# Inception3D/Motion324

Measured on AMD Instinct MI355X. Metric: frames/sec (32-frame clip, 2048 pts, 512x512), higher is better.
Workload: dtype bf16; 1 GPU; Motion_Latent_Model.forward inference, B=1 x 32 frames x 2048 points x 512x512 video, 4096 surface samples, training.frames=32, random-init weights (one clip per GPU; BASELINE configs[1]); the clip sits in the replayed graph's input buffers in HBM; bf16 speed mode with the decoder's residual stream in bf16 and the head fused (no [rows, C] intermediate) (secondary.headline_without_precision_shortcu; parallelism=clip-parallel x1

## Files before the change

### include/m324.h

```cpp
#ifndef M324_H
#define M324_H

#ifdef __cplusplus
extern "C" {
#endif

typedef enum { M324_OK = 0, M324_ERR_INVALID = -1, M324_ERR_HIP = -2, M324_ERR_UNSUPPORTED = -3 } m324_status;
typedef enum { M324_F32 = 0, M324_BF16 = 1, M324_MXFP8 = 2 } m324_dtype;
typedef enum { M324_ACT_NONE = 0, M324_ACT_GELU = 1 } m324_act;
typedef enum { M324_AUX_NONE = 0, M324_AUX_STORE_PREACT = 1, M324_AUX_MUL_GELU_GRAD = 2, M324_AUX_QKV_HEADS = 3,
               M324_AUX_QKV_HEADS_VT = 4, M324_AUX_N3 = 5, M324_AUX_STORE_GELU_GRAD = 6, M324_AUX_MUL = 7 } m324_aux_mode;

int m324_abi_version(void);
int m324_last_error(char* buf, int n);
int m324_device_info(char* name, int n);
int m324_set_tunable(const char* name, int value);

typedef struct {
    const void* A;  long lda;
    const void* W;  long ldw;
    void* C;        long ldc;
    int M, N, K;
    int in_dtype, out_dtype;
    const float* bias;
// ... 5 lines not shown
    long strideA, strideW, strideC;
    void* aux; long ldaux; int aux_mode;
    void* qkv_q; void* qkv_k; void* qkv_v;
    const float* qkv_qw; const float* qkv_kw;
    float qkv_eps, qkv_qscale;
    int qkv_L, qkv_H;
    const float* ln_rowstat; const float* ln_colsum;
    float* ln_stats_out;
    void* ln_copy_out; long ln_ldcopy;
    int ln_ncb; float ln_eps;
} m324_gemm_args;
int m324_gemm(const m324_gemm_args* a, void* stream);
int m324_gemm_pair(const m324_gemm_args* a, const m324_gemm_args* b, void* stream);
int m324_gemm_plan(const m324_gemm_args* a, char* buf, int n);

int m324_mx_quant(const void* x, int x_dtype, long ldx, int rows, int K, void* q, long ldq, void* s, long lds, void* stream);
int m324_layernorm_mx(const float* x, long ldx, const float* w, const float* b, float eps, int rows, int C, void* q, long ldq,
                      void* s, long lds, void* stream);
int m324_gemm_mx(const m324_gemm_args* a, const void* A_scale, long lds_a, const void* W_scale, long lds_w, void* C_scale,
                 long lds_c, void* stream);

int m324_rowstats_finish(const float* part, int ncb, int M, float eps, float* rowstat, void* stream);
int m324_rowstats(const float* x, long ldx, int rows, int C, float eps, float* rowstat, void* copy, long ldcopy, void* stream);

int m324_n3_finish(const float* part, int ncb, int M, const float* bias3, float* out, void* stream);

int m324_gemm_tn(const void* X, long ldx, const void* Y, long ldy, float* C, long ldc, int M, int N, int Kc,
                 int slices, long strideC, void* stream);

int m324_layernorm(const float* x, long ldx, const float* w, const float* b, float eps,
                   void* y, long ldy, int out_dtype, int rows, int C,
                   int gin, int gout, int off, void* stream);
int m324_layernorm_pair(const float* x0, long ldx0, const float* w0, const float* b0, float eps0, void* y0, long ldy0, int rows0,
                        int gin0, int gout0, int off0, const float* x1, long ldx1, const float* w1, const float* b1, float eps1,
                        void* y1, long ldy1, int rows1, int gin1, int gout1, int off1, int C, int out_dtype, void* stream);
int m324_layernorm_in(const void* x, int x_dtype, long ldx, const float* w, const float* b, float eps,
                      void* y, long ldy, int out_dtype, int rows, int C,
                      int gin, int gout, int off, void* stream);

int m324_qkv_split(const void* q_src, long ldq, const void* k_src, long ldk, const void* v_src, long ldv,
                   const float* q_w, const float* k_w, float eps, float q_scale,
                   void* Q, void* K, void* V, void* Qt, void* Kt, void* Vt,
                   int B, int L, int H, int dtype, void* stream);

enum { M324_ATTN_Q_PRESCALED = 1, M324_ATTN_V_ROWMAJOR = 2, M324_ATTN_SCORES_BOUNDED = 4 };
int m324_attention(const void* Q, long q_bstride, const void* K, const void* Vt, void* O, long ldo,
// ... 100 lines not shown
```

### motion324_amd/Pcd_motion.py

```python
from __future__ import annotations

import contextlib
import os

from typing import Dict, Optional

import torch
import torch.nn as nn
import torch.nn.functional as F

from . import ops, parallel, switches
from .easydict import EasyDict as edict
from .image_encoder import DINO_EPS, DinoEncoder
from .lib import ACT_GELU, M324Error
from .loss import MSELossComputer
from .prepared import Prepared, bump_generation, compute_dtype, pad_k
from .timing import span
from . import transformer as _transformer
from .transformer import (LN_EPS, LNFold, QK_Norm_CrossAttentionBlock, QK_Norm_TransformerBlock, fusion_off, init_weights,
                          mx_scope)

AUTO_GRAPH = switches.flag("M324_AUTO_GRAPH")
FUSE_HEAD_N3 = switches.flag("M324_FUSE_HEAD")
KV_REHEARSE = int(switches.get("M324_KV_REHEARSE") or 0)
KV_OVERLAP = switches.flag("M324_KV_OVERLAP")
BF16_DECODER_STREAM = switches.flag("M324_BF16_DECODER")
HOIST_DECODER_Q = switches.flag("M324_HOIST_Q")
DECODE_ROWS = int(switches.get("M324_DECODE_ROWS"))
MXFP8_DEFAULT = switches.flag("M324_MXFP8")


def _get(cfg, key, default=None):
    if isinstance(cfg, dict):
        return cfg.get(key, default)
    return getattr(cfg, key, default)


class PointEmbed(nn.Module):

    def __init__(self, hidden_dim=48, dim=768):
        super().__init__()
        if hidden_dim != 48:
            raise NotImplementedError("m324_point_encode implements the reference's 48 Fourier features")
        self.embedding_dim = hidden_dim
        e = torch.pow(2, torch.arange(hidden_dim // 6)).float() * torch.pi
        z = torch.zeros(hidden_dim // 6)
        self.register_buffer("basis", torch.stack([torch.cat([e, z, z]), torch.cat([z, e, z]), torch.cat([z, z, e])]))
        self.mlp = nn.Linear(hidden_dim + 3, dim)


def generate_pos_embed(T: int, H: int, W: int, embed_dim: int) -> torch.Tensor:
    def axis(n):
# ... 463 lines not shown
        drop_seed = int(torch.randint(0, 2 ** 62, (1,)).item()) if drop_p > 0.0 else 0
        pos = self._video_pos(P, T_full)[t0 * Pn:(t0 + T) * Pn]
        sp_rest = P.f32(self.special_token_rest).reshape(4, C)
        sp_first = P.f32(self.special_token_0).reshape(4, C) if t0 == 0 else sp_rest
        tok = ops.assemble_tokens(dino_x, P.vec(enc.norm.weight), P.vec(enc.norm.bias), DINO_EPS, pos, sp_first, sp_rest,
                                  mesh, P.vec(self.transformer_input_layernorm.weight),
                                  self.transformer_input_layernorm.eps, B, T, K, Pn, drop_p, drop_seed)
        Lt = 4 + K + Pn
        if cap is not None:
            dn = torch.empty((B * T * Pn, C), dtype=torch.float32, device=dev)
            ops.layernorm(dino_x, P.vec(enc.norm.weight), P.vec(enc.norm.bias), DINO_EPS, dn, row_map=(Pn, Pn + 1, 1))
            cap["dino_tokens"], cap["trunk_in"] = dn, tok.clone()

        if shard is not None and parallel.collectives_on(shard[1]):
            rank, world, group = shard[:3]
            kv_gather = _KVGather(B, T, Lt, parallel.counts(T_full, world), group, dev, rank=rank)

        fold = None
        if LNFold.usable(P, tok.shape[0], C) and "trunk.mlp" not in mx.roles:
            fold = LNFold(tok)
            if "trunk.qkv" not in mx.roles:
                fold.from_stream(tok, self.global_transformer_blocks[0].norm1.eps)
        n_pairs = len(self.global_transformer_blocks)
        for i, (gblk, lblk) in enumerate(zip(self.global_transformer_blocks, self.local_transformer_blocks)):
            with mx:
                gblk.run(P, tok, B, T * Lt, kv_gather=kv_gather, fold=fold)
                lblk.run(P, tok, B * T, Lt, fold=fold, feed_next=i + 1 < n_pairs)
            if cap is not None and "trunk_block0" not in cap:
                cap["trunk_block0"] = tok.clone()
        if cap is not None:
            cap["trunk_out"] = tok.clone()

        dec = self.decoder_cross_attn
        out = torch.empty((B, T, N, 3), dtype=torch.float32, device=dev)
        head_ln, head_fc1, head_fc2 = self.shared_mlp_output[0], self.shared_mlp_output[1], self.shared_mlp_output[3]
        w3, b3 = P.f32(head_fc2.weight), P.vec(head_fc2.bias)
        nchunk = max(1, min(N, DECODE_ROWS // T))
        pcd, nrm, rgb = (self._f32c(sample[k]) for k in ("ref_pcd", "ref_normal", "ref_rgb"))
        paired = None
        if hoisted is None and B == 1 and nchunk == N:
            pf0 = self._point_features(P, pcd[0], nrm[0].contiguous(), rgb[0].contiguous())
            with span("stage:decoder_cross_attn_block", self.decoder_block_flops(B, T, N)):
                Q0, Kd, Vd = dec.project_q_kv(P, pf0, N, tok, B * T, K, row_map=(K, Lt, 4))
            paired = (pf0, Q0)
        else:
            with span("stage:decoder_cross_attn_block", self.decoder_block_flops(B, T, N)):
                Kd, Vd = dec.project_kv(P, tok, B * T, K, row_map=(K, Lt, 4))
        for b in range(B):
            for n0 in range(0, N, nchunk):
                n1 = min(N, n0 + nchunk)
                if hoisted is not None:
                    pf, Q = hoisted[b]
                elif paired is not None:
                    pf, Q = paired
                else:
                    pf = self._point_features(P, pcd[b, n0:n1], nrm[b, n0:n1].contiguous(), rgb[b, n0:n1].contiguous())
                with span("stage:decoder_cross_attn_block", 0.0):
                    x, fold_d = self.decoder_block(P, Kd[b * T:(b + 1) * T], Vd[b * T:(b + 1) * T], pf,
                                                   None if (hoisted is None and paired is None) else Q)
                if cap is not None and n0 == 0 and n1 == N:
                    cap.setdefault("decoder_out_t0", []).append(x[:N].clone())
                if fold_d is not None:
                    hw, hcs, hb = P.folded(head_ln.weight, head_ln.bias, head_fc1.weight, head_fc1.bias)
                    h, lnk = fold_d.xb, dict(ln=fold_d.ln(head_ln.eps, hcs))
                else:
                    h = torch.empty(x.shape, dtype=P.dtype, device=dev)
                    ops.layernorm(x, P.vec(head_ln.weight), P.vec(head_ln.bias), head_ln.eps, h)
                    hw, hb, lnk = P.mat(head_fc1.weight), P.vec(head_fc1.bias), {}
                whole = n0 == 0 and n1 == N
                o = out[b] if whole else torch.empty((T, n1 - n0, 3), dtype=torch.float32, device=dev)
# ... 42 lines not shown
```

### motion324_amd/csrc/elementwise.hip

```cpp
#include "common.h"

namespace {

constexpr int LN_MAXV = 4;

__device__ __forceinline__ long remap_row(long r, int gin, int gout, int off) {
    return gin > 0 ? (r / gin) * gout + (r % gin) + off : r;
}

#define LN_FOR(i, c) _Pragma("unroll") for (int i = 0, c = lane * 4; i < LN_MAXV; ++i, c += 256) if (c < C)

__device__ __forceinline__ void row_load(float4 (&v)[LN_MAXV], const float* src, int lane, int C) {
    LN_FOR(i, c) v[i] = *reinterpret_cast<const float4*>(src + c);
}
__device__ __forceinline__ void row_stats(const float4 (&v)[LN_MAXV], int lane, int C, float eps, float& mean, float& rstd) {
    float s = 0.f;
    LN_FOR(i, c) s += v[i].x + v[i].y + v[i].z + v[i].w;
    mean = wave_sum(s) / (float)C;
    float q = 0.f;
    LN_FOR(i, c) {
        float a = v[i].x - mean, b = v[i].y - mean, cc = v[i].z - mean, d = v[i].w - mean;
        q += a * a + b * b + cc * cc + d * d;
    }
    rstd = rsqrtf(wave_sum(q) / (float)C + eps);
// ... 128 lines not shown
    const float n = 64.0f * (float)ncb, mean = s / n;
    float m2 = 0.f;
    for (int b = 0; b < ncb; ++b) {
        const float2 pb = part[(long)b * M + m];
        const float d = pb.x * (1.0f / 64.0f) - mean;
        m2 += fmaf(64.0f * d, d, pb.y);
    }
    const float rstd = rsqrtf(m2 / n + eps);
    rowstat[m] = make_float2(rstd, -rstd * mean);
}

__global__ __launch_bounds__(256) void rowstats_kernel(const float* __restrict__ x, long ldx, int rows, int C, float eps,
                                                       float2* __restrict__ rowstat, bf16_t* __restrict__ copy, long ldcopy) {
    const int lane = threadIdx.x & 63;
    const long row = (long)blockIdx.x * 4 + (threadIdx.x >> 6);
    if (row >= rows) return;
    float4 v[LN_MAXV];
    row_load(v, x + row * ldx, lane, C);
    float mean, rstd;
    row_stats(v, lane, C, eps, mean, rstd);
    if (lane == 0) rowstat[row] = make_float2(rstd, -rstd * mean);
    if (copy) {
        LN_FOR(i, c) store4<bf16_t>(copy + row * ldcopy + c, v[i].x, v[i].y, v[i].z, v[i].w);
    }
}

template <typename T>
__global__ __launch_bounds__(256) void qkv_split_kernel(const T* __restrict__ qs, long ldq, const T* __restrict__ ks, long ldk,
                                                        const T* __restrict__ vs, long ldv, const float* __restrict__ qw,
                                                        const float* __restrict__ kw, float eps, float q_scale,
                                                        T* __restrict__ Q, T* __restrict__ K, T* __restrict__ V,
                                                        T* __restrict__ Qt, T* __restrict__ Kt, T* __restrict__ Vt, int L, int H,
                                                        int Lp) {
    __shared__ float tile[64][65];
    const int t = threadIdx.x, tok = t >> 2, part = t & 3;
    const int b = blockIdx.z, h = blockIdx.y, l0 = blockIdx.x * 64;
    const int l = l0 + tok;
    const bool ok = l < L;
    const long srow = (long)b * L + l;
    const long hbase = ((long)b * H + h);

    auto one = [&](const T* src, long ld, const float* w, float post, T* dst, T* dstT) {
        float v[16];
        if (ok) {
            const T* p = src + srow * ld + h * 64 + part * 16;
            float lo[8], hi8[8];
// ... 698 lines not shown
    else M324_FAIL(M324_ERR_UNSUPPORTED, name ": dtype %d", (int)(dtype))

extern "C" int m324_rowstats_finish(const float* part, int ncb, int M, float eps, float* rowstat, void* stream) {
    M324_REQUIRE(part && rowstat && ncb > 0 && M > 0, "m324_rowstats_finish: bad arguments (ncb=%d M=%d)", ncb, M);
    M324_REQUIRE(((uintptr_t)part % 8) == 0 && ((uintptr_t)rowstat % 8) == 0, "m324_rowstats_finish: tables must be 8-byte aligned");
    hipLaunchKernelGGL(rowstats_finish_kernel, dim3(ceil_div(M, 256)), dim3(256), 0, (hipStream_t)stream,
                       reinterpret_cast<const float2*>(part), ncb, M, eps, reinterpret_cast<float2*>(rowstat));
    M324_CHECK_LAUNCH("m324_rowstats_finish");
    return M324_OK;
}

extern "C" int m324_rowstats(const float* x, long ldx, int rows, int C, float eps, float* rowstat, void* copy, long ldcopy,
                             void* stream) {
    M324_REQUIRE(x && rowstat && rows > 0, "m324_rowstats: bad arguments");
    M324_REQUIRE(C % 4 == 0 && C > 0 && C <= 256 * LN_MAXV && ldx % 4 == 0 && ldx >= C, "m324_rowstats: C=%d ldx=%ld unsupported", C, ldx);
    M324_REQUIRE(((uintptr_t)rowstat % 8) == 0 && (!copy || (ldcopy % 4 == 0 && ldcopy >= C && ((uintptr_t)copy % 8) == 0)),
                 "m324_rowstats: misaligned outputs");
    hipLaunchKernelGGL(rowstats_kernel, dim3(ceil_div(rows, 4)), dim3(256), 0, (hipStream_t)stream, x, ldx, rows, C, eps,
                       reinterpret_cast<float2*>(rowstat), static_cast<bf16_t*>(copy), ldcopy);
    M324_CHECK_LAUNCH("m324_rowstats");
    return M324_OK;
}

extern "C" int m324_layernorm_in(const void* x, int x_dtype, long ldx, const float* w, const float* b, float eps, void* y, long ldy,
                                 int out_dtype, int rows, int C, int gin, int gout, int off, void* stream) {
    if (x_dtype == M324_F32) return m324_layernorm((const float*)x, ldx, w, b, eps, y, ldy, out_dtype, rows, C, gin, gout, off, stream);
    M324_REQUIRE(x && w && y, "m324_layernorm_in: null pointer");
    M324_REQUIRE(x_dtype == M324_BF16 && out_dtype == M324_BF16, "m324_layernorm_in: a bf16 input needs a bf16 output");
    M324_REQUIRE(rows > 0 && C % 4 == 0 && C > 0 && C <= 256 * LN_MAXV && ldx % 4 == 0 && ldy % 4 == 0,
                 "m324_layernorm_in: rows=%d C=%d ldx=%ld ldy=%ld unsupported", rows, C, ldx, ldy);
    if (m324::tunable(m324::TUN_LN_ROWS) == 1)
        hipLaunchKernelGGL((layernorm1_kernel<bf16_t, bf16_t>), dim3(ceil_div(rows, 4)), dim3(256), 0, (hipStream_t)stream,
                           (const bf16_t*)x, ldx, w, b, eps, (bf16_t*)y, ldy, rows, C, gin, gout, off);
    else
    hipLaunchKernelGGL((layernorm_kernel<bf16_t, bf16_t>), dim3(ceil_div(rows, 8)), dim3(256), 0, (hipStream_t)stream,
                       (const bf16_t*)x, ldx, w, b, eps, (bf16_t*)y, ldy, rows, C, gin, gout, off);
    M324_CHECK_LAUNCH("m324_layernorm_in");
    return M324_OK;
}

extern "C" int m324_layernorm(const float* x, long ldx, const float* w, const float* b, float eps, void* y, long ldy,
                              int out_dtype, int rows, int C, int gin, int gout, int off, void* stream) {
    M324_REQUIRE(x && w && y, "m324_layernorm: null pointer");
    M324_REQUIRE(rows > 0, "m324_layernorm: rows=%d", rows);
    M324_REQUIRE(C % 4 == 0 && C > 0 && C <= 256 * LN_MAXV, "m324_layernorm: C=%d unsupported", C);
    M324_REQUIRE(ldx % 4 == 0 && ldy % 4 == 0, "m324_layernorm: leading dims must be multiples of 4");
// ... 384 lines not shown
```

### motion324_amd/lib.py

```python
from __future__ import annotations

import ctypes as C
import os
import threading

HERE = os.path.dirname(os.path.abspath(__file__))
LIB_PATH = os.environ.get("M324_LIB") or os.path.join(HERE, "libm324.so")

F32, BF16, MXFP8 = 0, 1, 2
ACT_NONE, ACT_GELU = 0, 1
ABI_VERSION = 23
ERR_UNSUPPORTED = -3


class M324Error(RuntimeError):
    pass


class GemmArgs(C.Structure):
    _fields_ = [
        ("A", C.c_void_p), ("lda", C.c_long),
        ("W", C.c_void_p), ("ldw", C.c_long),
        ("C", C.c_void_p), ("ldc", C.c_long),
        ("M", C.c_int), ("N", C.c_int), ("K", C.c_int),
# ... 23 lines not shown
class MirrorItem(C.Structure):
    _fields_ = [("src_off", C.c_long), ("dst_off", C.c_long), ("dstT_off", C.c_long), ("first_tile", C.c_long), ("rows", C.c_int),
                ("cols", C.c_int), ("ldT", C.c_int), ("pad_", C.c_int)]


_P, _L, _I, _F = C.c_void_p, C.c_long, C.c_int, C.c_float

SIGNATURES = {
    "m324_abi_version": [],
    "m324_last_error": [C.c_char_p, _I],
    "m324_device_info": [C.c_char_p, _I],
    "m324_set_tunable": [C.c_char_p, _I],
    "m324_gemm": [C.POINTER(GemmArgs), _P],
    "m324_gemm_plan": [C.POINTER(GemmArgs), C.c_char_p, _I],
    "m324_gemm_pair": [C.POINTER(GemmArgs), C.POINTER(GemmArgs), _P],
    "m324_mx_quant": [_P, _I, _L, _I, _I, _P, _L, _P, _L, _P],
    "m324_layernorm_mx": [_P, _L, _P, _P, _F, _I, _I, _P, _L, _P, _L, _P],
    "m324_gemm_mx": [C.POINTER(GemmArgs), _P, _L, _P, _L, _P, _L, _P],
    "m324_attention_plan": [_I, _I, _I, _I, _I, _I, C.c_char_p, _I],
    "m324_gemm_tn": [_P, _L, _P, _L, _P, _L, _I, _I, _I, _I, _L, _P],
    "m324_n3_finish": [_P, _I, _I, _P, _P, _P],
    "m324_rowstats_finish": [_P, _I, _I, _F, _P, _P],
    "m324_rowstats": [_P, _L, _I, _I, _F, _P, _P, _L, _P],
    "m324_layernorm": [_P, _L, _P, _P, _F, _P, _L, _I, _I, _I, _I, _I, _I, _P],
    "m324_layernorm_in": [_P, _I, _L, _P, _P, _F, _P, _L, _I, _I, _I, _I, _I, _I, _P],
    "m324_layernorm_pair": [_P, _L, _P, _P, _F, _P, _L, _I, _I, _I, _I, _P, _L, _P, _P, _F, _P, _L, _I, _I, _I, _I, _I, _I, _P],
    "m324_qkv_split": [_P, _L, _P, _L, _P, _L, _P, _P, _F, _F, _P, _P, _P, _P, _P, _P, _I, _I, _I, _I, _P],
    "m324_attention": [_P, _L, _P, _P, _P, _L, _I, _I, _I, _I, _F, _I, _P, _I, _P],
    "m324_attention_merge": [_P, _P, _P, _P, _P, _P, _L, _P, _L, _I, _I, _I, _I, _P],
    "m324_patchify": [_P, _I, _I, _I, _I, _I, _P, _I, _I, _P],
    "m324_patchify_u8": [_P, _I, _I, _I, _I, _I, _P, _I, _I, _P],
    "m324_point_encode": [_P, _I, _P, _L, _I, _P],
    "m324_point_concat": [_P, _P, _I, _P, _I, _I, _I, _P],
    "m324_dino_cls_rows": [_P, _P, _P, _I, _I, _I, _P],
    "m324_assemble_tokens": [_P, _P, _P, _F, _P, _P, _P, _P, _P, _F, _P, _I, _I, _I, _I, _I, _F, C.c_ulonglong, _P],
    "m324_linear_n3": [_P, _L, _P, _P, _P, _I, _I, _I, _P],
    "m324_mse": [_P, _P, _L, _F, _P, _P, _P],
    "m324_smooth_trajectories": [_P, _P, _P, _I, _I, _I, _F, _F, _P],
    "m324_smooth_savgol": [_P, _P, _I, _I, _I, _P, _I, _P],
    "m324_smooth_oneeuro": [_P, _P, _I, _I, _I, _F, _F, _F, _P],
    "m324_nearest_point": [_P, _I, _P, _I, _P, _P],
    "m324_transpose": [_P, _L, _P, _L, _I, _I, _I, _I, _P],
    "m324_colsum": [_P, _L, _P, _I, _I, _I, _I, _P, _I, _P],
    "m324_colsum_multi": [C.POINTER(ColsumItem), _I, _P],
    "m324_gelu": [_P, _P, _L, _I, _P],
    "m324_gelu_bwd": [_P, _P, _P, _L, _I, _P],
# ... 84 lines not shown
```

### motion324_amd/ops.py

```python
from __future__ import annotations

import ctypes as C
from typing import NamedTuple, Optional

import torch

from . import lib as L
from . import switches
from .timing import active as _timing, span

F32, BF16, MXFP8 = L.F32, L.BF16, L.MXFP8
_TORCH_DT = {F32: torch.float32, BF16: torch.bfloat16}


def code_of(dtype: torch.dtype) -> int:
    if dtype == torch.float32:
        return F32
    if dtype == torch.bfloat16:
        return BF16
    raise L.M324Error(f"unsupported dtype {dtype}")


def torch_dtype(code: int) -> torch.dtype:
    return _TORCH_DT[code]
# ... 376 lines not shown
    if (two != 2 or part.dtype != torch.float32 or not part.is_contiguous() or rowstat.dtype != torch.float32
            or not rowstat.is_contiguous() or rowstat.numel() != 2 * M):
        raise L.M324Error("rowstats_finish: part [ncb, M, 2] and rowstat [M, 2] must be contiguous fp32")
    with span("hbm_pass", 0.0, 8.0 * (ncb + 1) * M, f"rowstats_finish_kernel | rows={M} blocks={ncb}" if _timing() else ""):
        L.check(L.load().m324_rowstats_finish(_p(part), ncb, M, eps, _p(rowstat), _stream()), "m324_rowstats_finish")
    return rowstat


def rowstats(x: torch.Tensor, eps: float, rowstat: torch.Tensor, copy: Optional[torch.Tensor] = None) -> torch.Tensor:
    px, ldx = _rows(x, "x")
    rows, Cdim = x.shape
    if x.dtype != torch.float32 or rowstat.dtype != torch.float32 or not rowstat.is_contiguous() or rowstat.numel() != 2 * rows:
        raise L.M324Error("rowstats: x fp32 [rows, C], rowstat contiguous fp32 [rows, 2]")
    pc, ldc = (None, 0)
    if copy is not None:
        if copy.dtype != torch.bfloat16 or copy.shape[0] < rows or copy.shape[1] != Cdim:
            raise L.M324Error("rowstats: copy must be bf16 [rows, C]")
        pc, ldc = _rows(copy, "copy")
    with span("hbm_pass", 0.0, rows * Cdim * (4.0 + (2.0 if copy is not None else 0.0)), f"rowstats_kernel | rows={rows} C={Cdim}" if _timing() else ""):
        L.check(L.load().m324_rowstats(px, ldx, rows, Cdim, eps, _p(rowstat), pc, ldc, _stream()), "m324_rowstats")
    return rowstat


def layernorm(x: torch.Tensor, w: torch.Tensor, b: Optional[torch.Tensor], eps: float, out: torch.Tensor,
              rows: Optional[int] = None, row_map=(0, 0, 0)) -> torch.Tensor:
    if x.dtype != torch.float32 and not (x.dtype == torch.bfloat16 and out.dtype == torch.bfloat16):
        raise L.M324Error("layernorm: x must be fp32 (or bf16 with a bf16 output)")
    px, ldx = _rows(x, "x")
    py, ldy = _rows(out, "out")
    Cdim = x.shape[1]
    rows = out.shape[0] if rows is None else rows
    gin, gout, off = row_map
    need = ((rows - 1) // gin * gout + (rows - 1) % gin + off + 1) if gin > 0 else rows
    if x.shape[0] < need or out.shape[0] < rows or out.shape[1] != Cdim:
        raise L.M324Error("layernorm: shape mismatch")
    tag = (f"layernorm_kernel<{'unsigned short' if out.element_size() == 2 else 'float'}, {'unsigned short' if x.element_size() == 2 else 'float'}>"
           f" | rows={rows} C={Cdim}") if _timing() else ""
    with span("hbm_pass", 0.0, float(rows) * Cdim * (x.element_size() + out.element_size()), tag):
        if x.dtype == torch.bfloat16:
            L.check(L.load().m324_layernorm_in(px, BF16, ldx, _vec(w, Cdim, "w"), _vec(b, Cdim, "b"), eps, py, ldy, code_of(out.dtype),
                                               rows, Cdim, gin, gout, off, _stream()), "m324_layernorm_in")
        else:
            L.check(L.load().m324_layernorm(px, ldx, _vec(w, Cdim, "w"), _vec(b, Cdim, "b"), eps, py, ldy, code_of(out.dtype),
                                            rows, Cdim, gin, gout, off, _stream()), "m324_layernorm")
    return out

# ... 481 lines not shown
```

### motion324_amd/switches.py

```python
from __future__ import annotations

import os
from typing import Dict, Tuple

HOST: Dict[str, Tuple[str, str, str]] = {
    "M324_AUTO_GRAPH": ("1", "Pcd_motion.AUTO_GRAPH", "inference forward(): hipGraph replay from the third call with the same shapes on"),
    "M324_FUSE_HEAD": ("1", "Pcd_motion.FUSE_HEAD_N3", "bf16 inference: head Linear + GELU + Linear(C -> 3) in one GEMM epilogue (M324_AUX_N3)"),
    "M324_BF16_DECODER": ("1", "Pcd_motion.BF16_DECODER_STREAM", "bf16 inference: the decoder's two-addition residual stream in bf16 (0: fp32 like the trunk)"),
    "M324_HOIST_Q": ("1", "Pcd_motion.HOIST_DECODER_Q", "graph capture: decoder point features + q projection on the shape-encoder branch"),
    "M324_DECODE_ROWS": (str(1 << 17), "Pcd_motion.DECODE_ROWS", "max (frames x points) rows per decoder pass"),
    "M324_OVERLAP": ("1", "Pcd_motion.OVERLAP_SHAPE_ENCODER", "inference: shape encoder on a second HIP stream under the image encoder"),
    "M324_KV_OVERLAP": ("0", "Pcd_motion.KV_OVERLAP", "frame-parallel (one sample), opt-in until it has run on a multi-GPU RCCL node: 1 = every global block attends to the rank's own keys while the k|v all-gather is in flight, then to the gathered remote keys, and merges the partial softmaxes by their log-sum-exps (0: one attention after the gather)"),
    "M324_KV_REHEARSE": ("0", "Pcd_motion.KV_REHEARSE", "one rank with forced collectives (bench.py M324_BENCH_COLLECT=1): W > 1 runs every global block's overlapped form as rank 0 of W would (own keys = the first 1 / W of the frames), to price the split attention + merge on one GPU"),
    "M324_FOLD_LN": ("2", "transformer.FOLD_LN", "LayerNorm fold: 0 off, 1 bf16 streams only (the decoder), 2 every stream (trunk, DINO too)"),
    "M324_FOLD_MERGE": ("1", "transformer.FOLD_MERGE", "LayerNorm fold: the consumer GEMM merges the producer's per-block row statistics itself (0: m324_rowstats_finish launch between them)"),
    "M324_PAIR_PROJ": ("1", "transformer.PAIR_PROJ", "bf16 inference, decoder: norm_q + norm_kv in one launch and the q + k|v projections in one launch when the q projection runs inside the block (0: four launches)"),
    "M324_ATTN_BOUNDED": ("1", "transformer.ATTN_BOUNDED", "bf16 inference, long sequences: softmax without a reference maximum when the q / k RMSNorm weights bound every score (M324_ATTN_SCORES_BOUNDED)"),
    "M324_FUSE_QKV": ("1", "transformer.FUSE_QKV", "bf16 inference: q|k|v projection epilogue writes head-major Q / K / V (RMSNorm, pre-scale)"),
    "M324_FUSE_QKV_VT": ("1", "transformer.FUSE_QKV_VT", "the same for long sequences: the epilogue writes the transposed, key-permuted V"),
    "M324_TRAIN_STORE": ("1", "training.TRAIN_STORE", "training: the forward keeps block internals while they fit half of the free HBM (0: always recompute, the reference's checkpoint policy)"),
    "M324_TRAIN_DINO_FUSED": ("1", "training.DINO_FUSED", "training: the frozen DINOv2 encoder (no gradient flows through it) runs its inference form -- LayerNorm fold, fused q|k|v epilogue -- and is enqueued first in the step (0: the unfused form the trainable blocks use)"),
    "M324_DIRECT_GRADS": ("1", "backward.DIRECT_GRADS", "training: weight / bias gradients are written straight into the optimizer's flat gradient buffer (0: temporary + copy)"),
    "M324_ACC_GRADS": ("1", "backward.ACC_GRADS", "training: later gradients of a shared weight (the decoder's per-sample passes) are summed into the one it holds by the weight-gradient kernel's own reduction (0: temporary + torch add)"),
    "M324_GELU_GRAD_FWD": ("1", "backward.GELU_GRAD_FWD", "training: the fc1 GEMM of every MLP leaves gelu'(z) next to gelu(z) (M324_AUX_STORE_GELU_GRAD) and the dgrad GEMM behind fc2 multiplies by it (M324_AUX_MUL); 0: it leaves z and the dgrad epilogue evaluates erf and exp again"),
    "M324_WEIGHT_MIRROR": ("1", "optim.WEIGHT_MIRROR", "training: FusedAdamW keeps bf16 row-major and transposed copies of every Linear weight in two flat buffers, rewritten by one m324_weight_mirror launch after each update (0: Prepared casts / m324_transpose per weight and step)"),
    "M324_DEFER_COLSUM": ("1", "ops.DEFER_COLSUM", "training: the sums of the weight gradients' split-K partials and of the norm-weight partials wait in a queue and leave in one m324_colsum_multi launch per block (0: one m324_colsum launch each, at once)"),
    "M324_MXFP8": ("0", "Pcd_motion.MXFP8_DEFAULT", "1: a model whose config names no model.inference_precision uses \"mxfp8\" -- block-scaled e4m3 operands for the GEMM roles of transformer.MX_ROLES (the trunk and DINOv2 q|k|v projections) in a bf16 inference forward (DESIGN section 4)"),
    "M324_PRECISION": ("", "prepared.compute_dtype()", "force bf16 / fp32 (default: follow torch.autocast like the reference)"),
    "M324_LIB": ("", "lib.LIB_PATH", "path of an alternative libm324.so (lab builds)"),
    "M324_RCCL_LIB": ("", "csrc/comm.hip", "m324_comm_*: path of the RCCL library to bind (default: the copy already loaded, else librccl.so)"),
}
LIBRARY: Dict[str, Tuple[str, str]] = {
    "M324_GEMM": ("0", "force a GEMM schedule (v2 | v5 | v9 | v10 | v11 | v12 | v13 | v15); 0 = chooser"),
    "M324_GEMM_TN": ("0", "128: force the 128 x 128 weight-gradient kernel"),
    "M324_XCD": ("3", "tile order: bit 0 XCD-contiguous ranges (NN GEMMs; the weight-gradient GEMM's (slice, tile) items since round 6), bit 1 4 x 2 group order for wide weights, bit 2 force it; bit 3: the ring GEMMs' look-ahead pieces past the end of K fetch the last stage again (rounds 1-4) instead of nothing (A/B); bit 4: the 256 x 128 kernel (v12) without the residual prefetch (A/B)"),
    "M324_ATTN_NW": ("0", "attention forward: waves per workgroup (4 | 8); 0 = by sequence length"),
# ... 37 lines not shown
```

### motion324_amd/transformer.py

```python
from __future__ import annotations

import os

from typing import Optional

import torch
import torch.nn as nn

from . import ops, switches
from .lib import ACT_GELU
from .prepared import Prepared

LN_EPS = 1e-5
RMS_EPS = 1e-5


def init_weights(module, std=0.02):
    if isinstance(module, (nn.Linear, nn.Embedding)):
        torch.nn.init.normal_(module.weight, mean=0.0, std=std)
        if isinstance(module, nn.Linear) and module.bias is not None:
            torch.nn.init.zeros_(module.bias)


class RMSNorm(nn.Module):
    def __init__(self, dim: int, eps: float = RMS_EPS):
        super().__init__()
        self.eps = eps
        self.weight = nn.Parameter(torch.ones(dim))


class MLP(nn.Module):
    def __init__(self, dim, mlp_ratio=4, bias=False, dropout=0.0, activation=nn.GELU, mlp_dim=None):
        super().__init__()
# ... 176 lines not shown
    return role in _MX_ROLES_ON and not _FUSE_OFF and P.dtype == torch.bfloat16 and not torch.is_grad_enabled()


class fusion_allowed:

    def __enter__(self):
        global _FUSE_OFF
        self._saved, _FUSE_OFF = _FUSE_OFF, 0

    def __exit__(self, *exc):
        global _FUSE_OFF
        _FUSE_OFF = self._saved


def fuse_qkv(P: Prepared, rows: int, L: int) -> bool:
    return (FUSE_QKV and not _FUSE_OFF and P.dtype == torch.bfloat16 and rows > 64 and (L < 2048 or (FUSE_QKV_VT and L % 128 == 0))
            and not torch.is_grad_enabled())


def fuse_proj(P: Prepared, rows: int) -> bool:
    return FUSE_QKV and not _FUSE_OFF and P.dtype == torch.bfloat16 and rows > 64 and not torch.is_grad_enabled()


class QK_Norm_TransformerBlock(nn.Module):

    def __init__(self, dim, head_dim, ln_bias=False, attn_qkv_bias=False, attn_dropout=0.0, attn_fc_bias=False,
                 attn_fc_dropout=0.0, mlp_ratio=4, mlp_bias=False, mlp_dropout=0.0, use_qk_norm=True):
        super().__init__()
        self.norm1 = nn.LayerNorm(dim, bias=ln_bias)
        self.attn = QK_Norm_SelfAttention(dim, head_dim, qkv_bias=attn_qkv_bias, fc_bias=attn_fc_bias,
                                          attn_dropout=attn_dropout, fc_dropout=attn_fc_dropout, use_qk_norm=use_qk_norm)
        self.norm2 = nn.LayerNorm(dim, bias=ln_bias)
        self.mlp = MLP(dim, mlp_ratio=mlp_ratio, bias=mlp_bias, dropout=mlp_dropout)

    def run(self, P: Prepared, x: torch.Tensor, B: int, L: int, kv_gather=None, fold: Optional[LNFold] = None,
            feed_next: bool = True) -> torch.Tensor:
        rows, C = x.shape
        assert rows == B * L
        a = self.attn
        h = torch.empty((rows, C), dtype=P.dtype, device=x.device)
        qw, kw = a._qk_w(P)
        mx_qkv = kv_gather is None and mx_role(P, "trunk.qkv")
        mlp_mx = fold is None and mx_role(P, "trunk.mlp")
        proj = ops.gemm_mx if mx_qkv else ops.gemm
        if mx_qkv:
            src = ops.layernorm_mx(x, P.vec(self.norm1.weight), P.vec(self.norm1.bias), self.norm1.eps)
            w, bias = P.mx(a.to_qkv.weight), P.vec(a.to_qkv.bias)
            lnk = lambda lo, hi: {}
            feed_next = False
        elif fold is not None:
            w, cs, bias = P.folded(self.norm1.weight, self.norm1.bias, a.to_qkv.weight, a.to_qkv.bias)
            src, lnk = fold.xb, (lambda lo, hi: dict(ln=fold.ln(self.norm1.eps, cs[lo:hi])))
        else:
            ops.layernorm(x, P.vec(self.norm1.weight), P.vec(self.norm1.bias), self.norm1.eps, h)
            w, bias = P.mat(a.to_qkv.weight), P.vec(a.to_qkv.bias)
            src, lnk = h, (lambda lo, hi: {})
        out_kw = fold.producer if fold is not None else dict
        if fuse_qkv(P, rows, L) and kv_gather is None:
            long_seq = L >= 2048
            Q, K = (torch.empty((B, a.num_heads, L, 64), dtype=P.dtype, device=x.device) for _ in range(2))
            V = torch.empty((B, a.num_heads, 64, L) if long_seq else (B, a.num_heads, L, 64), dtype=P.dtype, device=x.device)
# ... 21 lines not shown
                def part(kv_rows, Lk):
                    _, Kp, Vp = ops.qkv_split(None, kv_rows[:, :C], kv_rows[:, C:], None, kw, RMS_EPS, B, Lk, H, P.dtype)
                    o = torch.empty((rows, C), dtype=P.dtype, device=x.device)
                    lse = torch.empty((B, H, L), dtype=torch.float32, device=x.device)
                    ops.attention(Q, Kp, Vp, o, prescaled=True, bounded=bounded, lse=lse)
                    return o, lse
                lo, hi = kv_gather.local_rows()
                own = kv[lo:hi] if getattr(kv_gather, "rehearse", 0) else kv
                parts = [part(own, hi - lo)]
                kv_full, L_full = kv_gather.finish()
                for r0, r1 in ((0, lo), (hi, L_full)):
                    if r1 > r0:
                        parts.append(part(kv_full[r0:r1], r1 - r0))
                ops.attention_merge(parts, h, B, H, L)
                ops.gemm(h, P.mat(a.fc.weight), x, bias=P.vec(a.fc.bias), residual=x, **out_kw())
                return _mlp_residual(P, self.norm2, self.mlp, x, fold, feed_next)
            kv_full, L_full = kv_gather.finish()
            _, K, Vt = ops.qkv_split(None, kv_full[:, :C], kv_full[:, C:], None, kw, RMS_EPS, B, L_full, a.num_heads,
                                     P.dtype)
        ops.attention(Q, K, Vt, h, prescaled=True, bounded=a.scores_bounded(P))
        ops.gemm(h, P.mat(a.fc.weight), x, bias=P.vec(a.fc.bias), residual=x, **out_kw())
        return _mlp_residual(P, self.norm2, self.mlp, x, fold, feed_next, mx=mlp_mx)

    def forward(self, x: torch.Tensor) -> torch.Tensor:
        B, L, C = x.shape
        P = Prepared.for_module(self, x.device)
        y = x.detach().float().reshape(B * L, C).clone()
        return self.run(P, y, B, L).reshape(B, L, C)


class QK_Norm_CrossAttentionBlock(nn.Module):

    def __init__(self, dim, head_dim, kv_dim=None, ln_bias=False, attn_qkv_bias=False, attn_dropout=0.0,
                 attn_fc_bias=False, attn_fc_dropout=0.0, mlp_ratio=4, mlp_bias=False, mlp_dropout=0.0, use_qk_norm=True):
        super().__init__()
        self.norm_q = nn.LayerNorm(dim, bias=ln_bias)
        self.norm_kv = nn.LayerNorm(kv_dim if kv_dim is not None else dim, bias=ln_bias)
        self.attn = QK_Norm_CrossAttention(dim, head_dim, kv_dim=kv_dim, qkv_bias=attn_qkv_bias, fc_bias=attn_fc_bias,
                                           attn_dropout=attn_dropout, fc_dropout=attn_fc_dropout, use_qk_norm=use_qk_norm)
        self.norm2 = nn.LayerNorm(dim, bias=ln_bias)
        self.mlp = MLP(dim, mlp_ratio=mlp_ratio, bias=mlp_bias, dropout=mlp_dropout)

    def project_q(self, P: Prepared, query: torch.Tensor, B: int, Lq: int) -> torch.Tensor:
        a = self.attn
        qn = torch.empty(query.shape, dtype=P.dtype, device=query.device)
        ops.layernorm(query, P.vec(self.norm_q.weight), P.vec(self.norm_q.bias), self.norm_q.eps, qn)
# ... 81 lines not shown
```

Baseline: 3560 frames/s.

## Prune trunk's last local block to latent rows the decoder reads

The final per-frame transformer block now computes k|v over all rows, then gathers only the latent rows of each frame (fp32 stream, bf16 twin and LayerNorm fold statistics) with a new gather kernel. It runs q projection, attention, out-projection and MLP on those rows only. The decoder then reads the compacted latent tensor instead of the full token stream. The aim is to skip query/MLP work on rows whose outputs are never consumed, at the cost of an extra gather launch and split k|v vs q GEMMs.

```diff
diff --git a/include/m324.h b/include/m324.h
--- a/include/m324.h
+++ b/include/m324.h
@@ -51,6 +51,9 @@
 
 int m324_rowstats_finish(const float* part, int ncb, int M, float eps, float* rowstat, void* stream);
 int m324_rowstats(const float* x, long ldx, int rows, int C, float eps, float* rowstat, void* copy, long ldcopy, void* stream);
+int m324_gather_stream_rows(const float* x, long ldx, float* x_out, long ldx_out, const void* xb, long ldxb, void* xb_out,
+                            long ldxb_out, const float* part, float* part_out, int ncb, int M_src, int rows, int C, int gin,
+                            int gout, int off, void* stream);
 
 int m324_n3_finish(const float* part, int ncb, int M, const float* bias3, float* out, void* stream);
 
diff --git a/motion324_amd/Pcd_motion.py b/motion324_amd/Pcd_motion.py
--- a/motion324_amd/Pcd_motion.py
+++ b/motion324_amd/Pcd_motion.py
@@ -18,7 +18,7 @@
 from .timing import span
 from . import transformer as _transformer
 from .transformer import (LN_EPS, LNFold, QK_Norm_CrossAttentionBlock, QK_Norm_TransformerBlock, fusion_off, init_weights,
-                          mx_scope)
+                          keep_rows_ok, mx_scope)
 
 AUTO_GRAPH = switches.flag("M324_AUTO_GRAPH")
 FUSE_HEAD_N3 = switches.flag("M324_FUSE_HEAD")
@@ -28,6 +28,7 @@
 HOIST_DECODER_Q = switches.flag("M324_HOIST_Q")
 DECODE_ROWS = int(switches.get("M324_DECODE_ROWS"))
 MXFP8_DEFAULT = switches.flag("M324_MXFP8")
+PRUNE_TAIL = switches.flag("M324_PRUNE_TAIL")
 
 
 def _get(cfg, key, default=None):
@@ -537,10 +538,18 @@
             if "trunk.qkv" not in mx.roles:
                 fold.from_stream(tok, self.global_transformer_blocks[0].norm1.eps)
         n_pairs = len(self.global_transformer_blocks)
+        latent_map = (K, Lt, 4)
+        prune = (PRUNE_TAIL and cap is None and n_pairs > 0 and not (mx.roles & {"trunk.qkv", "trunk.mlp"}) and B * T * K > 64
+                 and keep_rows_ok(P, B * T, Lt, C, latent_map, fold))
+        latent, latent_rows = tok, latent_map
         for i, (gblk, lblk) in enumerate(zip(self.global_transformer_blocks, self.local_transformer_blocks)):
+            last = i + 1 == n_pairs
             with mx:
                 gblk.run(P, tok, B, T * Lt, kv_gather=kv_gather, fold=fold)
-                lblk.run(P, tok, B * T, Lt, fold=fold, feed_next=i + 1 < n_pairs)
+                if last and prune:
+                    latent, latent_rows = lblk.run(P, tok, B * T, Lt, fold=fold, feed_next=False, keep=latent_map), (0, 0, 0)
+                else:
+                    lblk.run(P, tok, B * T, Lt, fold=fold, feed_next=not last)
             if cap is not None and "trunk_block0" not in cap:
                 cap["trunk_block0"] = tok.clone()
         if cap is not None:
@@ -556,11 +565,11 @@
         if hoisted is None and B == 1 and nchunk == N:
             pf0 = self._point_features(P, pcd[0], nrm[0].contiguous(), rgb[0].contiguous())
             with span("stage:decoder_cross_attn_block", self.decoder_block_flops(B, T, N)):
-                Q0, Kd, Vd = dec.project_q_kv(P, pf0, N, tok, B * T, K, row_map=(K, Lt, 4))
+                Q0, Kd, Vd = dec.project_q_kv(P, pf0, N, latent, B * T, K, row_map=latent_rows)
             paired = (pf0, Q0)
         else:
             with span("stage:decoder_cross_attn_block", self.decoder_block_flops(B, T, N)):
-                Kd, Vd = dec.project_kv(P, tok, B * T, K, row_map=(K, Lt, 4))
+                Kd, Vd = dec.project_kv(P, latent, B * T, K, row_map=latent_rows)
         for b in range(B):
             for n0 in range(0, N, nchunk):
                 n1 = min(N, n0 + nchunk)
diff --git a/motion324_amd/csrc/elementwise.hip b/motion324_amd/csrc/elementwise.hip
--- a/motion324_amd/csrc/elementwise.hip
+++ b/motion324_amd/csrc/elementwise.hip
@@ -174,6 +174,28 @@
     if (lane == 0) rowstat[row] = make_float2(rstd, -rstd * mean);
     if (copy) {
         LN_FOR(i, c) store4<bf16_t>(copy + row * ldcopy + c, v[i].x, v[i].y, v[i].z, v[i].w);
+    }
+}
+
+__global__ __launch_bounds__(256) void gather_stream_rows_kernel(const float* __restrict__ x, long ldx, float* __restrict__ xo, long ldxo,
+                                                                 const bf16_t* __restrict__ xb, long ldxb, bf16_t* __restrict__ xbo,
+                                                                 long ldxbo, const float2* __restrict__ part,
+                                                                 float2* __restrict__ parto, int ncb, int M_src, int rows, int C,
+                                                                 int gin, int gout, int off) {
+    const int lane = threadIdx.x & 63;
+    const long row = (long)blockIdx.x * 4 + (threadIdx.x >> 6);
+    if (row >= rows) return;
+    const long src = remap_row(row, gin, gout, off);
+    if (x) {
+        for (int c = lane * 4; c < C; c += 256)
+            *reinterpret_cast<float4*>(xo + row * ldxo + c) = *reinterpret_cast<const float4*>(x + src * ldx + c);
+    }
+    if (xb) {
+        for (int c = lane * 8; c < C; c += 512)
+            *reinterpret_cast<uint4*>(xbo + row * ldxbo + c) = *reinterpret_cast<const uint4*>(xb + src * ldxb + c);
+    }
+    if (part) {
+        for (int cb = lane; cb < ncb; cb += 64) parto[(long)cb * rows + row] = part[(long)cb * M_src + src];
     }
 }
 
@@ -918,6 +940,34 @@
     return M324_OK;
 }
 
+extern "C" int m324_gather_stream_rows(const float* x, long ldx, float* x_out, long ldx_out, const void* xb, long ldxb, void* xb_out,
+                                       long ldxb_out, const float* part, float* part_out, int ncb, int M_src, int rows, int C, int gin,
+                                       int gout, int off, void* stream) {
+    M324_REQUIRE((x != nullptr) == (x_out != nullptr) && (xb != nullptr) == (xb_out != nullptr) && (part != nullptr) == (part_out != nullptr),
+                 "m324_gather_stream_rows: every source needs its destination (and the reverse)");
+    M324_REQUIRE(x || xb || part, "m324_gather_stream_rows: nothing to gather");
+    M324_REQUIRE(rows > 0 && M_src > 0 && C > 0, "m324_gather_stream_rows: rows=%d M_src=%d C=%d", rows, M_src, C);
+    M324_REQUIRE(gin <= 0 || (off >= 0 && gout >= gin + off), "m324_gather_stream_rows: row map (%d, %d, %d): a group of gin rows at off must fit gout",
+                 gin, gout, off);
+    const long last = gin > 0 ? (long)((rows - 1) / gin) * gout + (rows - 1) % gin + off : rows - 1;
+    M324_REQUIRE(last < M_src, "m324_gather_stream_rows: row %ld of a source of %d rows", last, M_src);
+    M324_REQUIRE(!x || (C % 4 == 0 && ldx % 4 == 0 && ldx_out % 4 == 0 && ldx >= C && ldx_out >= C && ((uintptr_t)x % 16) == 0 &&
+                        ((uintptr_t)x_out % 16) == 0),
+                 "m324_gather_stream_rows: fp32 stream C=%d ldx=%ld ldx_out=%ld (16-byte rows)", C, ldx, ldx_out);
+    M324_REQUIRE(!xb || (C % 8 == 0 && ldxb % 8 == 0 && ldxb_out % 8 == 0 && ldxb >= C && ldxb_out >= C && ((uintptr_t)xb % 16) == 0 &&
+                         ((uintptr_t)xb_out % 16) == 0),
+                 "m324_gather_stream_rows: bf16 twin C=%d ldxb=%ld ldxb_out=%ld (16-byte rows)", C, ldxb, ldxb_out);
+    M324_REQUIRE(!part || (ncb > 0 && ((uintptr_t)part % 8) == 0 && ((uintptr_t)part_out % 8) == 0),
+                 "m324_gather_stream_rows: statistics tables must be 8-byte aligned, ncb=%d", ncb);
+    M324_REQUIRE((!x || x != x_out) && (!xb || xb != xb_out) && (!part || part != part_out),
+                 "m324_gather_stream_rows: in place is not supported");
+    hipLaunchKernelGGL(gather_stream_rows_kernel, dim3(ceil_div(rows, 4)), dim3(256), 0, (hipStream_t)stream, x, ldx, x_out, ldx_out,
+                       static_cast<const bf16_t*>(xb), ldxb, static_cast<bf16_t*>(xb_out), ldxb_out, reinterpret_cast<const float2*>(part),
+                       reinterpret_cast<float2*>(part_out), ncb, M_src, rows, C, gin, gout, off);
+    M324_CHECK_LAUNCH("m324_gather_stream_rows");
+    return M324_OK;
+}
+
 extern "C" int m324_layernorm_in(const void* x, int x_dtype, long ldx, const float* w, const float* b, float eps, void* y, long ldy,
                                  int out_dtype, int rows, int C, int gin, int gout, int off, void* stream) {
     if (x_dtype == M324_F32) return m324_layernorm((const float*)x, ldx, w, b, eps, y, ldy, out_dtype, rows, C, gin, gout, off, stream);
diff --git a/motion324_amd/lib.py b/motion324_amd/lib.py
--- a/motion324_amd/lib.py
+++ b/motion324_amd/lib.py
@@ -69,6 +69,7 @@
     "m324_n3_finish": [_P, _I, _I, _P, _P, _P],
     "m324_rowstats_finish": [_P, _I, _I, _F, _P, _P],
     "m324_rowstats": [_P, _L, _I, _I, _F, _P, _P, _L, _P],
+    "m324_gather_stream_rows": [_P, _L, _P, _L, _P, _L, _P, _L, _P, _P, _I, _I, _I, _I, _I, _I, _I, _P],
     "m324_layernorm": [_P, _L, _P, _P, _F, _P, _L, _I, _I, _I, _I, _I, _I, _P],
     "m324_layernorm_in": [_P, _I, _L, _P, _P, _F, _P, _L, _I, _I, _I, _I, _I, _I, _P],
     "m324_layernorm_pair": [_P, _L, _P, _P, _F, _P, _L, _I, _I, _I, _I, _P, _L, _P, _P, _F, _P, _L, _I, _I, _I, _I, _I, _I, _P],
diff --git a/motion324_amd/ops.py b/motion324_amd/ops.py
--- a/motion324_amd/ops.py
+++ b/motion324_amd/ops.py
@@ -422,6 +422,38 @@
     return rowstat
 
 
+def gather_stream_rows(rows: int, row_map, x: Optional[torch.Tensor] = None, x_out: Optional[torch.Tensor] = None,
+                       xb: Optional[torch.Tensor] = None, xb_out: Optional[torch.Tensor] = None,
+                       part: Optional[torch.Tensor] = None, part_out: Optional[torch.Tensor] = None) -> None:
+    gin, gout, off = row_map
+    given = [t for t in (x, xb, part) if t is not None]
+    if not given or (x is None) != (x_out is None) or (xb is None) != (xb_out is None) or (part is None) != (part_out is None):
+        raise L.M324Error("gather_stream_rows: sources and destinations come in pairs, at least one of them")
+    M = part.shape[1] if x is None and xb is None else given[0].shape[0]
+    Cdim = given[0].shape[1] if (x is not None or xb is not None) else 64 * part.shape[0]
+    (px, ldx), (pxo, ldxo), (pb, ldb), (pbo, ldbo) = ((None, 0),) * 4
+    if x is not None:
+        if x.dtype != torch.float32 or x_out.dtype != torch.float32 or tuple(x.shape) != (M, Cdim) or tuple(x_out.shape) != (rows, Cdim):
+            raise L.M324Error(f"gather_stream_rows: x {x.dtype}{tuple(x.shape)} -> x_out {x_out.dtype}{tuple(x_out.shape)} (want fp32 [{M}, {Cdim}] -> [{rows}, {Cdim}])")
+        (px, ldx), (pxo, ldxo) = _rows(x, "x"), _rows(x_out, "x_out")
+    if xb is not None:
+        if xb.dtype != torch.bfloat16 or xb_out.dtype != torch.bfloat16 or tuple(xb.shape) != (M, Cdim) or tuple(xb_out.shape) != (rows, Cdim):
+            raise L.M324Error(f"gather_stream_rows: xb {xb.dtype}{tuple(xb.shape)} -> xb_out {xb_out.dtype}{tuple(xb_out.shape)} (want bf16 [{M}, {Cdim}] -> [{rows}, {Cdim}])")
+        (pb, ldb), (pbo, ldbo) = _rows(xb, "xb"), _rows(xb_out, "xb_out")
+    ncb = 0
+    if part is not None:
+        ncb = part.shape[0]
+        if (part.dtype != torch.float32 or part_out.dtype != torch.float32 or not part.is_contiguous() or not part_out.is_contiguous()
+                or tuple(part.shape) != (ncb, M, 2) or tuple(part_out.shape) != (ncb, rows, 2)):
+            raise L.M324Error(f"gather_stream_rows: part {part.dtype}{tuple(part.shape)} -> part_out {part_out.dtype}{tuple(part_out.shape)} "
+                              f"(want contiguous fp32 [{ncb}, {M}, 2] -> [{ncb}, {rows}, 2])")
+    nbytes = 2.0 * rows * ((4 * Cdim if x is not None else 0) + (2 * Cdim if xb is not None else 0) + 8 * ncb)
+    with span("hbm_pass", 0.0, nbytes, f"gather_stream_rows_kernel | rows={rows} C={Cdim}" if _timing() else ""):
+        L.check(L.load().m324_gather_stream_rows(px, ldx, pxo, ldxo, pb, ldb, pbo, ldbo, _p(part), _p(part_out), ncb, M, rows, Cdim,
+                                                 gin, gout, off, _stream()), "m324_gather_stream_rows")
+    _wrote(x_out, xb_out, part_out)
+
+
 def layernorm(x: torch.Tensor, w: torch.Tensor, b: Optional[torch.Tensor], eps: float, out: torch.Tensor,
               rows: Optional[int] = None, row_map=(0, 0, 0)) -> torch.Tensor:
     if x.dtype != torch.float32 and not (x.dtype == torch.bfloat16 and out.dtype == torch.bfloat16):
diff --git a/motion324_amd/switches.py b/motion324_amd/switches.py
--- a/motion324_amd/switches.py
+++ b/motion324_amd/switches.py
@@ -12,6 +12,7 @@
     "M324_OVERLAP": ("1", "Pcd_motion.OVERLAP_SHAPE_ENCODER", "inference: shape encoder on a second HIP stream under the image encoder"),
     "M324_KV_OVERLAP": ("0", "Pcd_motion.KV_OVERLAP", "frame-parallel (one sample), opt-in until it has run on a multi-GPU RCCL node: 1 = every global block attends to the rank's own keys while the k|v all-gather is in flight, then to the gathered remote keys, and merges the partial softmaxes by their log-sum-exps (0: one attention after the gather)"),
     "M324_KV_REHEARSE": ("0", "Pcd_motion.KV_REHEARSE", "one rank with forced collectives (bench.py M324_BENCH_COLLECT=1): W > 1 runs every global block's overlapped form as rank 0 of W would (own keys = the first 1 / W of the frames), to price the split attention + merge on one GPU"),
+    "M324_PRUNE_TAIL": ("1", "Pcd_motion.PRUNE_TAIL", "folded bf16 inference: the trunk's last per-frame block projects q, attends and runs its out-projection and MLP on the latent rows of every frame only -- the rows the decoder reads -- after one m324_gather_stream_rows launch; k|v still cover every row (0: the whole block on every row; bit-identical)"),
     "M324_FOLD_LN": ("2", "transformer.FOLD_LN", "LayerNorm fold: 0 off, 1 bf16 streams only (the decoder), 2 every stream (trunk, DINO too)"),
     "M324_FOLD_MERGE": ("1", "transformer.FOLD_MERGE", "LayerNorm fold: the consumer GEMM merges the producer's per-block row statistics itself (0: m324_rowstats_finish launch between them)"),
     "M324_PAIR_PROJ": ("1", "transformer.PAIR_PROJ", "bf16 inference, decoder: norm_q + norm_kv in one launch and the q + k|v projections in one launch when the q projection runs inside the block (0: four launches)"),
diff --git a/motion324_amd/transformer.py b/motion324_amd/transformer.py
--- a/motion324_amd/transformer.py
+++ b/motion324_amd/transformer.py
@@ -8,7 +8,7 @@
 import torch.nn as nn
 
 from . import ops, switches
-from .lib import ACT_GELU
+from .lib import ACT_GELU, M324Error
 from .prepared import Prepared
 
 LN_EPS = 1e-5
@@ -231,6 +231,13 @@
     return FUSE_QKV and not _FUSE_OFF and P.dtype == torch.bfloat16 and rows > 64 and not torch.is_grad_enabled()
 
 
+def keep_rows_ok(P: Prepared, B: int, L: int, C: int, keep, fold: Optional[LNFold]) -> bool:
+    gin, gout, off = keep
+    return (fold is not None and fold.rows == B * L and 0 < gin and 0 <= off and gin + off <= L and gout == L and L < 2048
+            and fuse_qkv(P, B * L, L) and LNFold.usable(P, B * gin, C)
+            and not mx_role(P, "trunk.qkv") and not mx_role(P, "trunk.mlp"))
+
+
 class QK_Norm_TransformerBlock(nn.Module):
 
     def __init__(self, dim, head_dim, ln_bias=False, attn_qkv_bias=False, attn_dropout=0.0, attn_fc_bias=False,
@@ -243,9 +250,14 @@
         self.mlp = MLP(dim, mlp_ratio=mlp_ratio, bias=mlp_bias, dropout=mlp_dropout)
 
     def run(self, P: Prepared, x: torch.Tensor, B: int, L: int, kv_gather=None, fold: Optional[LNFold] = None,
-            feed_next: bool = True) -> torch.Tensor:
+            feed_next: bool = True, keep=None) -> torch.Tensor:
         rows, C = x.shape
         assert rows == B * L
+        if keep is not None:
+            if kv_gather is not None or not keep_rows_ok(P, B, L, C, keep, fold):
+                raise M324Error(f"QK_Norm_TransformerBlock.run: keep={tuple(keep)} needs the folded bf16 inference path of a short-sequence "
+                                f"block with more than 64 rows to keep (B={B} L={L} C={C}); ask keep_rows_ok() first")
+            return self._run_kept(P, x, B, L, keep, fold)
         a = self.attn
         h = torch.empty((rows, C), dtype=P.dtype, device=x.device)
         qw, kw = a._qk_w(P)
@@ -313,6 +325,29 @@
         ops.gemm(h, P.mat(a.fc.weight), x, bias=P.vec(a.fc.bias), residual=x, **out_kw())
         return _mlp_residual(P, self.norm2, self.mlp, x, fold, feed_next, mx=mlp_mx)
 
+    def _run_kept(self, P: Prepared, x: torch.Tensor, B: int, L: int, keep, fold: LNFold) -> torch.Tensor:
+        gin, gout, off = keep
+        rows, C = x.shape
+        a = self.attn
+        H, dev, kept = a.num_heads, x.device, B * gin
+        qw, kw = a._qk_w(P)
+        w, cs, bias = P.folded(self.norm1.weight, self.norm1.bias, a.to_qkv.weight, a.to_qkv.bias)
+        Kh, Vh = (torch.empty((B, H, L, 64), dtype=P.dtype, device=dev) for _ in range(2))
+        ops.gemm(fold.xb, w[C:], None, bias=None if bias is None else bias[C:],
+                 qkv_heads=(None, Kh, Vh, None, kw, RMS_EPS, ops.Q_PRESCALE, L, H, False), ln=fold.ln(self.norm1.eps, cs[C:]))
+        xk = torch.empty((kept, C), dtype=torch.float32, device=dev)
+        fk = LNFold(xk)
+        fk.pending = fold.pending
+        table, table_k = (fold.part, fk.part) if fold.pending else (fold.stat.view(1, rows, 2), fk.stat.view(1, kept, 2))
+        ops.gather_stream_rows(kept, keep, x=x, x_out=xk, xb=fold.xb, xb_out=fk.xb, part=table, part_out=table_k)
+        Qh = torch.empty((B, H, gin, 64), dtype=P.dtype, device=dev)
+        ops.gemm(fk.xb, w[:C], None, bias=None if bias is None else bias[:C],
+                 qkv_heads=(Qh, None, None, qw, None, RMS_EPS, ops.Q_PRESCALE, gin, H), ln=fk.ln(self.norm1.eps, cs[:C]))
+        o = torch.empty((kept, C), dtype=P.dtype, device=dev)
+        ops.attention(Qh, Kh, Vh, o, prescaled=True, v_rowmajor=True)
+        ops.gemm(o, P.mat(a.fc.weight), xk, bias=P.vec(a.fc.bias), residual=xk, **fk.producer())
+        return _mlp_residual(P, self.norm2, self.mlp, xk, fk, feed_next=False)
+
     def forward(self, x: torch.Tensor) -> torch.Tensor:
         B, L, C = x.shape
         P = Prepared.for_module(self, x.device)
```

New measurement: 3591 frames/s, median of 6. Within noise of the previous version (+0.9%).
